# gautam-sabnis/A-Divide-and-Conquer-Strategy-for-High-Dimensional-Bayesian-Factor-Models

Hardware: AMD Instinct MI355X
Metric: Gibbs iters/sec (node) at p=20k,n=1k,g=64; cov-assembly MFMA util % (higher is better)
Workload: dtype f64; 1 GPU; c3: p=19968 (P=312 x g=64), n=1000, K=30 (k=1920), rho=0.5, thin=5, burnin=0 (assembly in timed region), asm_batch=96; global_batch=1000, parallelism=shards64/gpus1

## Files before the change

a-divide-and-conquer-strategy-for-high-dimensional-bayesian-factor-models_amd/csrc/assemble.hip:

```cpp
#include "dcfm_internal.h"
#include "linalg.h"

#include <algorithm>

namespace dcfm {

template <bool M2>
__global__ __launch_bounds__(256) void k_save(Dims d, const double *__restrict__ Lam,
                                              const double *__restrict__ omega,
                                              double *__restrict__ Lb, double *__restrict__ wsum,
                                              int LDB, int slot, double *__restrict__ wslot, int B) {
    const size_t total = (size_t)d.G * d.P * d.K;
    for (size_t e = blockIdx.x * (size_t)blockDim.x + threadIdx.x; e < total;
         e += (size_t)gridDim.x * blockDim.x) {
        const int k = e % d.K;
        const size_t jm = e / d.K;
        const int j = jm % d.P, m = jm / d.P;
        const size_t a = (size_t)(d.shard0 + m) * d.P + j;
        Lb[a * LDB + (size_t)slot * d.K + k] = Lam[((size_t)m * d.PP + j) * d.kp + k];
        if (k == 0) {
            const double w = omega[(size_t)m * d.PP + j];
            wsum[a] += w;
            if (M2) wslot[a * B + slot] = w;
        }
    }
}

constexpr int AKC = ASM_KC, ALD = ASM_TILE + 16, ASM_THREADS = 256;

__device__ __forceinline__ void assemble_tile(const Dims &d, const double *__restrict__ Lb, int LDB, int kext,
                                              const double *__restrict__ wsum, double inv_eff, int2 T, int T0,
                                              double *__restrict__ Sig, double (*As)[AKC][ALD],
                                              double (*Bs)[AKC][ALD], int (*shard_of)[ASM_TILE]) {
    double *__restrict__ St = Sig + (size_t)(tri(T.x) - tri(T0) + T.y) * ASM_TILE * ASM_TILE;
    const int t = threadIdx.x, wave = t >> 6, lane = t & 63;
    shard_of[t >> 7][t & 127] = ((t < ASM_TILE ? T.x : T.y) * ASM_TILE + (t & 127)) / d.P;
    const int r = lane & 15, q = lane >> 4;
    const int p = d.p;
    const int wa = (wave >> 1) * 64, wb = (wave & 1) * 64;
    const int clast = min(p, T.y * ASM_TILE + ASM_TILE) - 1;
    const bool cross = (T.x * ASM_TILE) / d.P > clast / d.P;
    const double sA = cross ? d.rho * inv_eff : 1.0;
    const int srow = t >> 1, shalf = t & 1;
    const int ga = T.x * ASM_TILE + srow, gb = T.y * ASM_TILE + srow;
    const bool va = ga < p, vb = gb < p;
    const double *pa = Lb + (size_t)(va ? ga : 0) * LDB + 8 * shalf;
    const double *pb = Lb + (size_t)(vb ? gb : 0) * LDB + 8 * shalf;
    const d2 zero2 = {0.0, 0.0};
    d2 ra[4], rb[4];
    auto gload = [&](int kc) {
#pragma unroll
        for (int i = 0; i < 4; ++i) {
            ra[i] = va ? *reinterpret_cast<const d2 *>(pa + kc + 2 * i) : zero2;
            rb[i] = vb ? *reinterpret_cast<const d2 *>(pb + kc + 2 * i) : zero2;
        }
    };
    auto lstore = [&](int buf) {
#pragma unroll
        for (int i = 0; i < 4; ++i) {
            const int k = 8 * shalf + 2 * i;
            As[buf][k][srow] = sA * ra[i].x;
            As[buf][k + 1][srow] = sA * ra[i].y;
            Bs[buf][k][srow] = rb[i].x;
            Bs[buf][k + 1][srow] = rb[i].y;
        }
    };
    gload(0);
    d4 acc[4][4];
    auto sl = [&](int u, int v, int h) { return reinterpret_cast<d2 *>(St + sig_tile_off(u, v, 2 * h, wave, lane)); };
    if (cross) {
#pragma unroll
        for (int u = 0; u < 4; ++u)
#pragma unroll
            for (int v = 0; v < 4; ++v)
#pragma unroll
                for (int h = 0; h < 2; ++h) {
                    const d2 o = __builtin_nontemporal_load(sl(u, v, h));
                    acc[u][v][2 * h] = o.x;
                    acc[u][v][2 * h + 1] = o.y;
                }
    } else {
#pragma unroll
        for (int u = 0; u < 4; ++u)
#pragma unroll
            for (int v = 0; v < 4; ++v) acc[u][v] = d4{0.0, 0.0, 0.0, 0.0};
    }
    lstore(0);
    __syncthreads();
    for (int kc = 0, buf = 0; kc < kext; kc += AKC, buf ^= 1) {
        const bool more = kc + AKC < kext;
        if (more) gload(kc + AKC);
        const int nk4 = min(AKC, kext - kc);
#pragma unroll
        for (int s4 = 0; s4 < AKC / 4; ++s4) {
            if (4 * s4 >= nk4) break;
            double a[4], b[4];
#pragma unroll
            for (int u = 0; u < 4; ++u) a[u] = As[buf][4 * s4 + q][wa + 16 * u + r];
#pragma unroll
            for (int v = 0; v < 4; ++v) b[v] = Bs[buf][4 * s4 + q][wb + 16 * v + r];
#pragma unroll
            for (int u = 0; u < 4; ++u)
#pragma unroll
                for (int v = 0; v < 4; ++v) acc[u][v] = mfma16x16x4(a[u], b[v], acc[u][v]);
        }
        if (more) lstore(buf ^ 1);
        __syncthreads();
    }
    if (cross) {
#pragma unroll
        for (int u = 0; u < 4; ++u)
#pragma unroll
            for (int v = 0; v < 4; ++v)
#pragma unroll
                for (int h = 0; h < 2; ++h) {
                    d2 o;
                    o.x = acc[u][v][2 * h];
                    o.y = acc[u][v][2 * h + 1];
                    __builtin_nontemporal_store(o, sl(u, v, h));
                }
        return;
    }
    const int a0 = T.x * ASM_TILE + wa, b0 = T.y * ASM_TILE + wb;
    int sb[4];
#pragma unroll
    for (int v = 0; v < 4; ++v) sb[v] = shard_of[1][wb + 16 * v + r];
#pragma unroll
    for (int u = 0; u < 4; ++u) {
        double old[4][4];
#pragma unroll
        for (int g = 0; g < 4; ++g) {
            const int a = a0 + 16 * u + q + 4 * g;
#pragma unroll
            for (int v = 0; v < 4; ++v) {
                const int b = b0 + 16 * v + r;
                const bool live = a < p && b <= a;
                old[g][v] = live ? __builtin_nontemporal_load(&St[sig_tile_off(u, v, g, wave, lane)]) : 0.0;
            }
        }
#pragma unroll
        for (int g = 0; g < 4; ++g) {
            const int a = a0 + 16 * u + q + 4 * g;
            const int sa = shard_of[0][wa + 16 * u + q + 4 * g];
            const double dg = (a < p) ? wsum[a] * inv_eff : 0.0;
#pragma unroll
            for (int v = 0; v < 4; ++v) {
                const int b = b0 + 16 * v + r;
                if (a < p && b <= a) {
                    const double coef = (sb[v] == sa) ? 1.0 : d.rho;
                    double val = coef * acc[u][v][g] * inv_eff;
                    if (a == b) val += dg;
                    __builtin_nontemporal_store(old[g][v] + val, &St[sig_tile_off(u, v, g, wave, lane)]);
                }
            }
        }
    }
}

__global__ __launch_bounds__(256, 2) void k_assemble(Dims d, const double *__restrict__ Lb, int LDB,
                                                     int kext, const double *__restrict__ wsum,
                                                     double inv_eff, const int2 *__restrict__ tiles, int T0,
                                                     double *__restrict__ Sig) {
    __shared__ double As[2][AKC][ALD], Bs[2][AKC][ALD];
    __shared__ int shard_of[2][ASM_TILE];
    assemble_tile(d, Lb, LDB, kext, wsum, inv_eff, tiles[xcd_remap(blockIdx.x, gridDim.x)], T0, Sig, As, Bs,
                  shard_of);
}

template <int WHICH>
__global__ __launch_bounds__(256) void k_sigma_pack(const double *__restrict__ S, const double *__restrict__ S2,
                                                    double rs, int p, int T0, int T1, int c0, int nc,
                                                    double *__restrict__ out, int dset, double dval) {
    auto at = [&](size_t o) {
        if (WHICH == 0) return S[o];
        if (WHICH == 1) return S2[o];
        const double m = rs * S[o];
        return sqrt(fmax(0.0, fma(rs, S2[o], -m * m)));
    };
    __shared__ double lo[32][33];
    const int R0 = min(p, T0 * ASM_TILE), R1 = min(p, T1 * ASM_TILE);
    const int r0 = blockIdx.x * 32, cb = c0 + blockIdx.y * 32;
    const int tx = threadIdx.x & 31, ty = threadIdx.x >> 5;
    const bool need_lo = r0 + 31 >= cb;
    const bool need_up = r0 < cb + 31;
    if (need_lo) {
        for (int yy = ty; yy < 32; yy += 8) {
            const int r = r0 + yy, c = cb + tx;
            lo[yy][tx] = (r >= R0 && r < R1 && c < c0 + nc && r >= c) ? ((dset && r == c) ? dval : at(sig_off(r, c, T0))) : 0.0;
        }
    }
    __syncthreads();
    for (int yy = ty; yy < 32; yy += 8) {
        const int c = cb + yy, r = r0 + tx;
        if (c >= c0 + nc || r >= R1) continue;
        const long long wl = win_lo(c, R0, R1);
        if (r < wl) continue;
        const double v = (r >= c) ? lo[tx][yy] : (need_up ? at(sig_off(c, r, T0)) : 0.0);
        out[win_off(c, c0, R0, R1) + (r - wl)] = v;
    }
}

__global__ __launch_bounds__(256) void k_sigma_unpack(const double *__restrict__ recv, int p, int c0, int cbeg,
                                                      const int *__restrict__ Tb,
                                                      const long long *__restrict__ base, int nranks,
                                                      double *__restrict__ out) {
    const int c = cbeg + blockIdx.y;
    for (int r = blockIdx.x * 256 + threadIdx.x; r < p; r += gridDim.x * 256) {
        const int t = max(r, c) / ASM_TILE;
        int k = 0;
        while (k + 1 < nranks && Tb[k + 1] <= t) ++k;
        const long long R0 = min(p, Tb[k] * ASM_TILE), R1 = min(p, Tb[k + 1] * ASM_TILE);
        out[(size_t)(c - c0) * p + r] = recv[base[k] + win_off(c, c0, R0, R1) + (r - win_lo(c, R0, R1))];
    }
}

void launch_save(const Dims &d, const Bufs &b, double *Lb, double *wsum, int slot, hipStream_t s, double *wslot,
                 int B) {
    const size_t total = (size_t)d.G * d.P * d.K;
    const int grid = (int)std::min<size_t>((total + 255) / 256, 4096);
    if (wslot)
        hipLaunchKernelGGL(k_save<true>, dim3(grid), dim3(256), 0, s, d, b.Lam, b.omega, Lb, wsum, b.LDB, slot, wslot, B);
    else
        hipLaunchKernelGGL(k_save<false>, dim3(grid), dim3(256), 0, s, d, b.Lam, b.omega, Lb, wsum, b.LDB, slot, wslot, B);
}
void launch_assemble(const Dims &d, const Bufs &b, const double *Lb, const double *wsum, int kext,
                     double inv_eff, hipStream_t s) {
    if (b.ntiles == 0) return;
    hipLaunchKernelGGL(k_assemble, dim3(b.ntiles), dim3(ASM_THREADS), 0, s, d, Lb, b.LDB, kext, wsum, inv_eff,
                       b.tiles, b.T0, b.Sigma);
}
void launch_sigma_pack(const double *S, const double *S2, int which, double rs, int p, int T0, int T1, int c0,
                       int nc, double *out, hipStream_t s, const double *diag) {
    const int R1 = std::min(p, T1 * ASM_TILE);
    if (nc <= 0 || R1 <= 0 || T1 <= T0) return;
    const dim3 grid(cdiv(R1, 32), cdiv(nc, 32));
    const int dset = diag ? 1 : 0;
    const double dval = diag ? *diag : 0.0;
    if (which == 0)
        hipLaunchKernelGGL(k_sigma_pack<0>, grid, dim3(256), 0, s, S, S2, rs, p, T0, T1, c0, nc, out, dset, dval);
    else if (which == 1)
        hipLaunchKernelGGL(k_sigma_pack<1>, grid, dim3(256), 0, s, S, S2, rs, p, T0, T1, c0, nc, out, dset, dval);
    else hipLaunchKernelGGL(k_sigma_pack<2>, grid, dim3(256), 0, s, S, S2, rs, p, T0, T1, c0, nc, out, dset, dval);
}
void launch_sigma_unpack(const double *recv, int p, int c0, int nc, const int *Tb, const long long *base,
                         int nranks, double *out, hipStream_t s) {
    for (int j = 0; j < nc; j += 32768) {
        const int w = std::min(32768, nc - j);
        hipLaunchKernelGGL(k_sigma_unpack, dim3(std::min(cdiv(p, 256), 16), w), dim3(256), 0, s, recv, p, c0, c0 + j,
                           Tb, base, nranks, out);
    }
}

}
```

Measured before the change: 5719 iter/s.

## Software-pipeline LDS operand loads and staging in covariance assembly MFMA loop

Restructures the assembly GEMM inner loop so LDS operand reads for the next k-step are double-buffered in registers and overlap the current MFMAs. The next chunk's LDS staging moves to a configurable step inside the chunk, with a single barrier before switching buffers. Global loads become unconditional, with out-of-range rows zeroed at LDS-store time instead of via predicated loads. This aims to hide LDS and global latency behind MFMA work, at the cost of more registers. It also loads clamped row-0 data for invalid rows, which is safe but wastes some bandwidth.

```diff
diff --git a/a-divide-and-conquer-strategy-for-high-dimensional-bayesian-factor-models_amd/csrc/assemble.hip b/a-divide-and-conquer-strategy-for-high-dimensional-bayesian-factor-models_amd/csrc/assemble.hip
--- a/a-divide-and-conquer-strategy-for-high-dimensional-bayesian-factor-models_amd/csrc/assemble.hip
+++ b/a-divide-and-conquer-strategy-for-high-dimensional-bayesian-factor-models_amd/csrc/assemble.hip
@@ -27,6 +27,16 @@
 }
 
 constexpr int AKC = ASM_KC, ALD = ASM_TILE + 16, ASM_THREADS = 256;
+#ifndef DCFM_ASM_PIPE
+#define DCFM_ASM_PIPE 1
+#endif
+#ifndef DCFM_ASM_GLB
+#define DCFM_ASM_GLB 1
+#endif
+constexpr bool ASM_GLB = DCFM_ASM_GLB;
+#ifndef DCFM_ASM_LSTORE_AT
+#define DCFM_ASM_LSTORE_AT 2
+#endif
 
 __device__ __forceinline__ void assemble_tile(const Dims &d, const double *__restrict__ Lb, int LDB, int kext,
                                               const double *__restrict__ wsum, double inv_eff, int2 T, int T0,
@@ -51,18 +61,23 @@
     auto gload = [&](int kc) {
 #pragma unroll
         for (int i = 0; i < 4; ++i) {
-            ra[i] = va ? *reinterpret_cast<const d2 *>(pa + kc + 2 * i) : zero2;
-            rb[i] = vb ? *reinterpret_cast<const d2 *>(pb + kc + 2 * i) : zero2;
+            if (ASM_GLB) {
+                ra[i] = *reinterpret_cast<const d2 *>(pa + kc + 2 * i);
+                rb[i] = *reinterpret_cast<const d2 *>(pb + kc + 2 * i);
+            } else {
+                ra[i] = va ? *reinterpret_cast<const d2 *>(pa + kc + 2 * i) : zero2;
+                rb[i] = vb ? *reinterpret_cast<const d2 *>(pb + kc + 2 * i) : zero2;
+            }
         }
     };
     auto lstore = [&](int buf) {
 #pragma unroll
         for (int i = 0; i < 4; ++i) {
             const int k = 8 * shalf + 2 * i;
-            As[buf][k][srow] = sA * ra[i].x;
-            As[buf][k + 1][srow] = sA * ra[i].y;
-            Bs[buf][k][srow] = rb[i].x;
-            Bs[buf][k + 1][srow] = rb[i].y;
+            As[buf][k][srow] = ASM_GLB && !va ? 0.0 : sA * ra[i].x;
+            As[buf][k + 1][srow] = ASM_GLB && !va ? 0.0 : sA * ra[i].y;
+            Bs[buf][k][srow] = ASM_GLB && !vb ? 0.0 : rb[i].x;
+            Bs[buf][k + 1][srow] = ASM_GLB && !vb ? 0.0 : rb[i].y;
         }
     };
     gload(0);
@@ -87,6 +102,55 @@
     }
     lstore(0);
     __syncthreads();
+    auto opload = [&](int buf, int s4, double (&a)[4], double (&b)[4]) {
+#pragma unroll
+        for (int u = 0; u < 4; ++u) a[u] = As[buf][4 * s4 + q][wa + 16 * u + r];
+#pragma unroll
+        for (int v = 0; v < 4; ++v) b[v] = Bs[buf][4 * s4 + q][wb + 16 * v + r];
+    };
+    auto mma = [&](const double (&a)[4], const double (&b)[4]) {
+#pragma unroll
+        for (int u = 0; u < 4; ++u)
+#pragma unroll
+            for (int v = 0; v < 4; ++v) acc[u][v] = mfma16x16x4(a[u], b[v], acc[u][v]);
+    };
+#if DCFM_ASM_PIPE
+    constexpr int NS = AKC / 4, LAT = DCFM_ASM_LSTORE_AT;
+    static_assert(1 <= LAT && LAT < NS, "the staging precedes the chunk's barrier");
+    const int nch = (kext + AKC - 1) / AKC;
+    const int nlast = (kext - (nch - 1) * AKC) / 4;
+    double a[2][4], b[2][4];
+    int buf = 0;
+    opload(0, 0, a[0], b[0]);
+    for (int c = 0; c < nch - 1; ++c, buf ^= 1) {
+        gload((c + 1) * AKC);
+#pragma unroll
+        for (int s4 = 0; s4 < NS; ++s4) {
+            if (s4 + 1 < NS) {
+                opload(buf, s4 + 1, a[(s4 + 1) & 1], b[(s4 + 1) & 1]);
+            } else {
+                __builtin_amdgcn_sched_barrier(0);
+                __syncthreads();
+                opload(buf ^ 1, 0, a[0], b[0]);
+                __builtin_amdgcn_sched_barrier(0);
+            }
+            mma(a[s4 & 1], b[s4 & 1]);
+            if (s4 + 1 == LAT) {
+                __builtin_amdgcn_sched_barrier(0);
+#pragma unroll
+                for (int i = 0; i < 4; ++i) asm volatile("" : "+v"(ra[i]), "+v"(rb[i]));
+                lstore(buf ^ 1);
+            }
+        }
+    }
+    mma(a[0], b[0]);
+#pragma unroll
+    for (int s4 = 1; s4 < NS; ++s4) {
+        if (s4 >= nlast) break;
+        opload(buf, s4, a[1], b[1]);
+        mma(a[1], b[1]);
+    }
+#else
     for (int kc = 0, buf = 0; kc < kext; kc += AKC, buf ^= 1) {
         const bool more = kc + AKC < kext;
         if (more) gload(kc + AKC);
@@ -95,18 +159,13 @@
         for (int s4 = 0; s4 < AKC / 4; ++s4) {
             if (4 * s4 >= nk4) break;
             double a[4], b[4];
-#pragma unroll
-            for (int u = 0; u < 4; ++u) a[u] = As[buf][4 * s4 + q][wa + 16 * u + r];
-#pragma unroll
-            for (int v = 0; v < 4; ++v) b[v] = Bs[buf][4 * s4 + q][wb + 16 * v + r];
-#pragma unroll
-            for (int u = 0; u < 4; ++u)
-#pragma unroll
-                for (int v = 0; v < 4; ++v) acc[u][v] = mfma16x16x4(a[u], b[v], acc[u][v]);
+            opload(buf, s4, a, b);
+            mma(a, b);
         }
         if (more) lstore(buf ^ 1);
         __syncthreads();
     }
+#endif
     if (cross) {
 #pragma unroll
         for (int u = 0; u < 4; ++u)
```

After: 5845 iter/s (median of 6 runs). +2.2%, better.
